# brantburnett/Snappier

Hardware: AMD Instinct MI355X
Metric: uncompressed GB/s block compress+decompress, 64 KiB blocks (higher is better)
Workload: dtype u8

## Files before the change

### snappier_amd/csrc/decode_chains.hip

```cpp
#include "decode_common.h"

#define SNP_MARK(name) asm volatile("; MARK " #name)

#ifndef SNP_DC_FINISH_MIN
#define SNP_DC_FINISH_MIN 1
#endif

namespace {

constexpr u32 kR = 32;
constexpr u32 kW = SNP_WAVE * kR;
constexpr u32 kCap = 128;
constexpr u32 kModeBatch = 0, kModeWindow = 1, kModeLongLiteral = 2, kModeLeave = 3;
constexpr u32 kHist = 64;
constexpr u32 kStage = 2048;

__device__ __forceinline__ u32 adv4(u32 x)
{
    const u32 k1 = 0x01010101u;
    const u32 t = x & 0x03030303u;
    const u32 t1 = t >> 1;
    const u32 hp = ((x >> 2) & 0x3f3f3f3fu) + 0x02020202u;
    const u32 ca = t + k1 + (t1 & t & k1);
    const u32 nz = ((t | t1) & k1) * 255u;
    return (ca & nz) | (hp & ~nz);
}

__device__ __forceinline__ u32x4 adv16(u32x4 v) { return u32x4{adv4(v.x), adv4(v.y), adv4(v.z), adv4(v.w)}; }

__device__ __forceinline__ u32 long_literal_advance(const u8* at, u32 a)
{
    const u32 ex = a - 61u;
    const u32 b1234 = ld32u(at + 1);
    const u32 tr = ex >= 4 ? b1234 : __builtin_amdgcn_ubfe(b1234, 0u, 8 * ex);
    return 2u + ex + min(tr, 0x3fffffffu);
}

__device__ __forceinline__ void store_first_piece(u8* d, u32x4 p0, u32 len)
{
    if (len >= 16u) {
        st128u(d, p0);
    } else {
        const bool c8 = (len & 8u) != 0, c4 = (len & 4u) != 0, c2 = (len & 2u) != 0;
        const u32 a0 = c8 ? p0.z : p0.x;
        const u32 a1 = c8 ? p0.w : p0.y;
        const u32 b0 = c4 ? a1 : a0;
        const u32 c0 = c2 ? b0 >> 16 : b0;
        if (c8) st64u(d, p0.x, p0.y);
        if (c4) st32u(d + (len & 8u), a0);
        if (c2) st16u(d + (len & 12u), b0);
        if (len & 1u) d[len & 14u] = static_cast<u8>(c0);
    }
}

__device__ __forceinline__ void load_pieces(const u8* s, u32 len, bool any_mid, u32x4& p0, u32x4& p1, u32x4& p2, u32x4& p3)
{
    p0 = ld128u(s);
    if (len > 16u) p1 = ld128u(s + len - 16);
    if (any_mid) {
        if (len > 32u) {
            p2 = ld128u(s + 16);
            p3 = ld128u(s + min(32u, len - 16u));
        }
    }
}

__device__ __forceinline__ void store_pieces(u8* d, u32 len, bool any_mid, const u32x4& p0, const u32x4& p1, const u32x4& p2, const u32x4& p3)
{
    store_first_piece(d, p0, len);
    if (len > 16u) st128u(d + len - 16, p1);
    if (any_mid) {
        if (len > 32u) {
            st128u(d + 16, p2);
            if (len > 48u) st128u(d + 32, p3);
        }
    }
}

template <bool FENCED, bool FRAG>
__device__ __forceinline__ void chains_front(DecBlk& B, const u32 lane)
{
    __shared__ __attribute__((aligned(16))) u8 c_tab[kW + 64];
    __shared__ __attribute__((aligned(16))) u8 c_stage_h[kHist + kStage + 64];
    __shared__ u64 c_busy[65];
    u8* const c_stage = c_stage_h + kHist;
    u32* const c_T = reinterpret_cast<u32*>(c_busy);
    u16* const c_pos = reinterpret_cast<u16*>(c_tab);
    const u8* const src = B.src;
    u8* const dst = B.dst;
    const u32 n = B.n, expected = B.expected;
    const u32 skip = FRAG ? B.skip : 0u;
    u32 op = B.op;
    const u32 r0 = kR * lane;
    u32 wbase = B.ip, ntok = 0, emitted = 0, consumed = 0;
    u32 q_pf = 0;
    u32 pf_at = ~0u;
    bool h_valid = false;
    u64 h_pend = 0;
    u32 h_pk = 0, h_op = 0, h_span = 0, h_hist = 0;
    auto finish_held = [&](const bool fence) __attribute__((always_inline)) {
        lanes_sync_lds();
        if (h_pend) {
            if (FENCED && fence) asm volatile("s_waitcnt vmcnt(0)" ::: "memory");
            const u32 vbase = lane + static_cast<u32>(reinterpret_cast<uintptr_t>(c_stage));
            const u32 vbase0 = vbase - lane;
            (void)vbase0;
            u64 pend = h_pend;
            while (pend) {
                u32 f, k;
#if SNP_DC_FINISH_MIN
                {
                    u32 t0, t1, t2, va, vb, vi;
                    asm volatile(
                        "1:\n\t"
                        "s_ff1_i32_b64 %[f], %[pend]\n\t"
                        "v_readlane_b32 %[k], %[pk], %[f]\n\t"
                        "s_bitset0_b64 %[pend], %[f]\n\t"
                        "s_cmp_lt_i32 %[k], 0\n\t"
                        "s_cbranch_scc1 2f\n\t"
                        "s_bfe_u32 %[t0], %[k], 0x7000b\n\t"
                        "s_lshr_b32 %[t1], %[k], 18\n\t"
                        "s_and_b32 %[t2], %[k], 0x7ff\n\t"
                        "v_min_u32_e32 %[vi], %[t0], %[lane]\n\t"
                        "v_add3_u32 %[va], %[vi], %[t1], %[vsrc]\n\t"
                        "ds_read_u8 %[vb], %[va]\n\t"
                        "v_add3_u32 %[va], %[vi], %[t2], %[vbase]\n\t"
                        "s_waitcnt lgkmcnt(0)\n\t"
                        "ds_write_b8 %[va], %[vb]\n\t"
                        "s_cmp_lg_u64 %[pend], 0\n\t"
                        "s_cbranch_scc1 1b\n\t"
                        "2:"
                        : [pend] "+s"(pend), [f] "=&s"(f), [k] "=&s"(k), [t0] "=&s"(t0), [t1] "=&s"(t1), [t2] "=&s"(t2),
                          [va] "=&v"(va), [vb] "=&v"(vb), [vi] "=&v"(vi)
                        : [pk] "v"(h_pk), [lane] "v"(lane), [vbase] "v"(vbase0), [vsrc] "v"(vbase0 - kHist)
                        : "scc", "memory");
#else
                {
                    u32 t0, t1, t2, va, vb;
                    u64 sv;
                    asm volatile(
                        "1:\n\t"
                        "s_ff1_i32_b64 %[f], %[pend]\n\t"
                        "v_readlane_b32 %[k], %[pk], %[f]\n\t"
                        "s_bitset0_b64 %[pend], %[f]\n\t"
                        "s_cmp_lt_i32 %[k], 0\n\t"
                        "s_cbranch_scc1 2f\n\t"
                        "s_bfe_u32 %[t0], %[k], 0x7000b\n\t"
                        "s_lshr_b32 %[t1], %[k], 18\n\t"
                        "s_and_b32 %[t2], %[k], 0x7ff\n\t"
                        "v_cmp_gt_u32_e32 vcc, %[t0], %[lane]\n\t"
                        "s_and_saveexec_b64 %[sv], vcc\n\t"
                        "v_add_u32_e32 %[va], %[t1], %[vsrc]\n\t"
                        "ds_read_u8 %[vb], %[va]\n\t"
                        "v_add_u32_e32 %[va], %[t2], %[vbase]\n\t"
                        "s_waitcnt lgkmcnt(0)\n\t"
                        "ds_write_b8 %[va], %[vb]\n\t"
                        "s_mov_b64 exec, %[sv]\n\t"
                        "s_cmp_lg_u64 %[pend], 0\n\t"
                        "s_cbranch_scc1 1b\n\t"
                        "2:"
                        : [pend] "+s"(pend), [f] "=&s"(f), [k] "=&s"(k), [t0] "=&s"(t0), [t1] "=&s"(t1), [t2] "=&s"(t2), [sv] "=&s"(sv),
                          [va] "=&v"(va), [vb] "=&v"(vb)
                        : [pk] "v"(h_pk), [lane] "v"(lane), [vbase] "v"(vbase), [vsrc] "v"(vbase - kHist)
                        : "vcc", "scc", "memory");
#endif
                    if (static_cast<i32>(k) >= 0) break;
                }
                const u32 f_d = k & 0x7ffu, f_len = ((k >> 11) & 0x7fu) + (SNP_DC_FINISH_MIN ? 1u : 0u);
                const u32 f_off = (k >> 18) & 0x1fffu;
                const u32 sidx = f_off < f_len ? lane_mod(lane, f_off) : lane;
                const u32 spos = f_d + sidx - f_off;
                u32 byte = 0;
                if (__builtin_expect(static_cast<i32>(f_d - f_off) >= -static_cast<i32>(h_hist), 1)) {
                    if (lane < f_len) byte = c_stage[static_cast<i32>(spos)];
                } else {
                    const bool below = static_cast<i32>(spos) < -static_cast<i32>(h_hist);
                    if ((lane < f_len) & !below) byte = c_stage[static_cast<i32>(spos)];
                    if ((lane < f_len) & below) byte = dst[h_op + spos];
                    asm volatile("" : "+v"(byte));
                }
                if (lane < f_len) c_stage[f_d + lane] = static_cast<u8>(byte);
                lanes_sync_lds();
            }
        }
    };
    auto write_out_held = [&]() __attribute__((always_inline)) {
        lanes_sync_lds();
        u8* const g = dst + h_op;
        if (FRAG && h_op < skip) {
            for (u32 i = skip - h_op + lane; i < h_span; i += SNP_WAVE) g[i] = c_stage[i];
        } else {
            for (u32 i = lane * 16; i < h_span; i += SNP_WAVE * 16)
                *reinterpret_cast<snp_u128_unaligned*>(g + i) = *reinterpret_cast<const snp_u128_unaligned*>(c_stage + i);
        }
    };
    for (;;) {
        u32 mode = emitted == ntok ? kModeWindow : kModeBatch;
        u32 len = 0, off = 0, drel = 0, ne = 0, incl = 0, body = 0, s_first = 0, s_len0 = 0, s_body0 = 0, taken = 0;
        bool is_lit = false, live = true;
        if (mode == kModeBatch) {
SNP_MARK(B_top);
            const u32 t = emitted + lane;
            bool have = t < ntok;
            const u32 pos = c_pos[have ? t : emitted];
            u32 q = q_pf;
            if (pf_at != emitted) {
                q = ld32u(src + wbase + pos);
                asm volatile("" : "+v"(q));
            }
            const u32 c = q & 0xffu;
            const u32 type = c & 3u;
            const u32 hi6 = c >> 2;
            u32 b1234 = q >> 8;
            if (__builtin_expect(ballot64(have & ((type == 3u) | (c == 0xfcu))) != 0ull, 0)) {
                if ((type == 3u) | (c == 0xfcu)) b1234 |= static_cast<u32>(src[wbase + pos + 4u]) << 24;
            }
            is_lit = type == 0;
            const bool long_lit = is_lit && hi6 >= 60;
            const u32 extra = is_lit ? (long_lit ? hi6 - 59 : 0u) : (type == 3 ? 4u : type);
            const u32 trailer = extra >= 4 ? b1234 : __builtin_amdgcn_ubfe(b1234, 0u, 8 * extra);
            len = (long_lit ? trailer : (hi6 & (type == 1 ? 7u : 63u))) + (type == 1 ? 4u : 1u);
            off = is_lit ? 0u : (type == 1 ? (((c >> 5) << 8) | (b1234 & 0xffu)) : trailer);
            body = pos + 1u + extra;
            u64 last = ~0ull;
            u32 len_tag0 = 0;
            bool dealt = false;
            if (!FRAG && __builtin_expect(ballot64((q & 0xc0ffu) == 0x40f0u) != 0ull, 0)) {
                const bool two = have && is_lit && len > 64u && len <= 128u;
                dealt = true;
                len_tag0 = read_lane(len, 0);
                const u32 cnt = have ? (two ? 2u : 1u) : 0u;
                const u32 sincl = wave_inclusive_scan(cnt);
                const u32 s0 = sincl - cnt;
                const bool fits = have && sincl <= SNP_WAVE;
                const u32 nslots = read_lane(sincl, static_cast<u32>(__builtin_popcountll(ballot64(fits))) - 1u);
                if (fits) c_busy[s0] = (two ? 64u : min(len, 255u)) | (two ? 0u : 0x100u) | (is_lit ? 0x200u : 0u) | (static_cast<u64>(body) << 10) | (static_cast<u64>(off) << 26);
                if (fits && two) c_busy[s0 + 1u] = (len - 64u) | 0x100u | 0x200u | (static_cast<u64>(body + 64u) << 10);
                lanes_sync_lds();
                const u64 w = c_busy[lane];
                lanes_sync_lds();
                have = lane < nslots;
                len = static_cast<u32>(w) & 0xffu;
                is_lit = (w & 0x200u) != 0;
                body = static_cast<u32>(w >> 10) & 0xffffu;
                off = static_cast<u32>(w >> 26);
                last = ballot64(have && (w & 0x100u) != 0) | ~ballot64(have);
            }
            const u32 olen = have ? len : 0u;
            incl = wave_inclusive_scan(olen);
            drel = incl - olen;
            const u32 room = n - wbase - 16u;
            const bool lit_ok = ((len - 1u) < room) & (body <= room - len);
            const bool dead = FRAG && op + incl <= skip;
            live = !FRAG || op + drel >= skip;
            const bool copy_ok = (off - 1u) < op + drel - skip;
            const bool ok = have & (dead ? (!is_lit | lit_ok) : live & ((is_lit & lit_ok) | (!is_lit & copy_ok))) & (incl + 16u <= expected - op);
            const bool big = is_lit & (len > 64u);
            const u64 okm = ballot64(ok & !big & (incl <= kStage));
            ne = okm == ~0ull ? 64u : static_cast<u32>(__builtin_ctzll(~okm));
            taken = ne;
            if (dealt) {
                if (ne && !((last >> (ne - 1u)) & 1ull)) ne -= 1u;
                taken = static_cast<u32>(__builtin_popcountll(last & (ne == 64u ? ~0ull : (1ull << ne) - 1ull)));
            }
SNP_MARK(B_ne0);
            if (ne == 0) {
                const u32 body0 = read_lane(body, 0);
                const bool long0 = dealt && read_lane(is_lit ? 1u : 0u, 0) != 0u && len_tag0 > 64u;
                const bool whole_ok = (len_tag0 - 1u) < room && body0 <= room - len_tag0 && static_cast<u64>(len_tag0) + 16u <= expected - op;
                const u32 f0 = long0 ? (whole_ok ? 3u : 0u) : read_lane((ok ? 1u : 0u) | (big ? 2u : 0u), 0);
                mode = f0 == 3u ? kModeLongLiteral : kModeLeave;
                s_first = read_lane(pos, 0);
                s_len0 = dealt ? len_tag0 : read_lane(len, 0);
                s_body0 = read_lane(body, 0) | (FRAG && read_lane(dead ? 1u : 0u, 0) ? 0x80000000u : 0u);
            }
        }
        if (mode != kModeBatch) {
            if (h_valid) {
                finish_held(true);
                write_out_held();
                h_valid = false;
            }
            if (mode == kModeLeave) {
                wbase += s_first;
                consumed = 0;
                break;
            }
            if (mode == kModeLongLiteral) {
                if (!FRAG || static_cast<i32>(s_body0) >= 0) wave_copy(dst + op, src + wbase + (s_body0 & 0x7fffffffu), s_len0, lane);
                op += s_len0;
                emitted += 1;
                continue;
            }
SNP_MARK(S_stage_table);
            wbase += consumed;
            consumed = 0;
            if (wbase + 72 > n || op >= expected) break;
            const u32 avail = n - wbase;
            const u32 L = min(kW, avail) - 8u;
            const u8* const wsrc = src + wbase;
            {
                const u32 oa = lane * 16u, ob = oa + 1024u;
                const u32 la = min(oa, avail - 16u), lb = min(ob, avail - 16u);
                const u32x4 va = ld128u(wsrc + la), vb = ld128u(wsrc + lb);
                st128u(c_tab + la, adv16(va));
                st128u(c_tab + lb, adv16(vb));
                lanes_sync_lds();
                c_tab[L + lane] = 64;
            }
            lanes_sync_lds();
SNP_MARK(A_walk);
            u32 p = r0, V = 0, a = 0;
            const u32 lim = min(r0 + kR, L);
            while (p < lim) {
                a = c_tab[p];
                c_tab[p] = static_cast<u8>(a | 0x80u);
                V |= 1u << (p & 31u);
                p += a;
            }
SNP_MARK(Aprime_walk);
            c_T[lane] = 0;
            u32* const c_O = reinterpret_cast<u32*>(c_stage + 512) + lane * (kCap / 32);
#pragma unroll
            for (u32 w = 0; w < kCap / 32; ++w) c_O[w] = 0;
            lanes_sync_lds();
            const bool stopA = (p > r0) & (a >= 62u);
            p = stopA ? p - a : min(p, L + 63u);
            const u32 obase = p & ~(kR - 1u);
            u32* const c_Ob = c_O - (obase >> 5);
            a = c_tab[p];
            u32 x = a | ((p - obase) & ~(kCap - 1u));
            while (x < 62u) {
                atomicOr(&c_Ob[p >> 5], 1u << (p & 31u));
                p += a;
                a = c_tab[p];
                x = a | ((p - obase) & ~(kCap - 1u));
            }
            const u32 nx = stopA ? 65u : (a & 0x80u) ? p >> 5 : (p >= L ? 64u : 65u);
SNP_MARK(R_reach);
            const u32 m = p;
            u64 active;
            u32 entry = 0;
            {
                u8* const c_reach = c_stage;
                u32* const c_entry = reinterpret_cast<u32*>(c_stage + SNP_WAVE);
                u32 hop = nx;
                bool reached = lane == 0;
                c_reach[lane] = reached ? 1 : 0;
#pragma unroll
                for (int k = 0; k < 6; ++k) {
                    lanes_sync_lds();
                    if (reached && hop < 64u) c_reach[hop] = 1;
                    lanes_sync_lds();
                    reached = c_reach[lane] != 0;
                    const u32 h2 = bperm(hop, hop);
                    hop = hop < 64u ? h2 : hop;
                }
                if (reached && nx < 64u) c_entry[nx] = m;
                lanes_sync_lds();
                if (lane) entry = c_entry[lane];
                lanes_sync_lds();
                active = ballot64(reached);
                const u64 ends = ballot64(reached && nx == 64u);
                consumed = ends ? read_lane(m, static_cast<u32>(__builtin_ctzll(ends))) : 0u;
            }
            if (ballot64(((active >> lane) & 1ull) && nx == 65u)) {
                active = 0;
                entry = 0;
                for (u32 k = 0, e = 0;;) {
                    active |= 1ull << k;
                    entry = lane == k ? e : entry;
                    u32 mk = read_lane(m, k), nk = read_lane(nx, k);
                    if (nk == 65u) {
                        nk = 64u;
                        for (bool first = true; mk < L; first = false) {
                            u32 a = bcast_first(static_cast<u32>(c_tab[mk]));
                            if (!first && a >= 128u) { nk = mk >> 5; break; }
                            a &= 0x7fu;
                            if (lane == 0) atomicOr(&c_T[mk >> 5], 1u << (mk & 31u));
                            if (a >= 62u) a = bcast_first(long_literal_advance(wsrc + mk, a));
                            mk += a;
                        }
                    }
                    if (nk >= 64u) { consumed = mk; break; }
                    e = mk;
                    k = nk;
                }
            }
SNP_MARK(T_list);
            if ((active >> lane) & 1ull) {
                const u32 own = V & ~((1u << (entry & 31u)) - 1u);
                const u32 w0 = obase >> 5;
                if (own) atomicOr(&c_T[lane], own);
#pragma unroll
                for (u32 w = 0; w < kCap / 32; ++w) {
                    const u32 ow = c_O[w];
                    if (ow && w0 + w < SNP_WAVE) atomicOr(&c_T[w0 + w], ow);
                }
            }
            lanes_sync_lds();
            const u32 Tw = c_T[lane];
            const u32 cnt = static_cast<u32>(__builtin_popcount(Tw));
            const u32 cincl = wave_inclusive_scan(cnt);
            ntok = read_lane(cincl, 63);
            lanes_sync_lds();
            u32 t = cincl - cnt, bits = Tw;
            while (bits) {
                c_pos[t++] = static_cast<u16>(r0 + static_cast<u32>(__builtin_ctz(bits)));
                bits &= bits - 1u;
            }
            lanes_sync_lds();
            emitted = 0;
            pf_at = ~0u;
            if (ntok == 0) {
                consumed = 0;
                break;
            }
            continue;
    }
SNP_MARK(B_pass1);
        const bool act = lane < ne;
        const u32 span = read_lane(incl, ne - 1);
        const u32 gap = h_valid ? op - h_op : 0u;
        const u32 reach = drel + len;
        const u32 back = gap + (h_valid ? h_hist : 0u);
        const bool far = !is_lit & (off >= reach + gap);
        const bool near = act & live & !is_lit & !far & (off >= reach) & (off <= drel + back);
        const bool early = act & live & (is_lit | far);
        const bool waits = act & live & !early & !near;
        if (FENCED) asm volatile("s_waitcnt vmcnt(0)" ::: "memory");
        pf_at = emitted + taken;
        if (pf_at < ntok) q_pf = ld32u(src + wbase + c_pos[pf_at + lane < ntok ? pf_at + lane : pf_at]);
        const bool any_mid = ballot64(act & (len > 32u)) != 0ull;
        const u32 sofs_mine = is_lit ? wbase + body : op + drel - off;
        u32x4 p0, p1, p2, p3;
        if (early) load_pieces((is_lit ? src : dst) + sofs_mine, len, any_mid, p0, p1, p2, p3);
SNP_MARK(B_finish);
        if (h_valid) finish_held(false);
SNP_MARK(B_writeout);
        asm volatile("; loads of the new batch are back"
                     :: "v"(p0.x), "v"(p0.y), "v"(p0.z), "v"(p0.w), "v"(p1.x), "v"(p1.y), "v"(p1.z), "v"(p1.w), "v"(p2.x), "v"(p2.y), "v"(p2.z),
                        "v"(p2.w), "v"(p3.x), "v"(p3.y), "v"(p3.z), "v"(p3.w), "v"(q_pf)
                     : "memory");
        if (h_valid) write_out_held();
SNP_MARK(B_stage);
        if (near) load_pieces(c_stage + static_cast<i32>(drel + gap - off), len, any_mid, p0, p1, p2, p3);
        const u32 hist = h_valid ? min(kHist, h_hist + gap) : 0u;
        if (hist) {
            const u8 hb = c_stage[static_cast<i32>(gap + lane - kHist)];
            if (lane >= kHist - hist) c_stage[static_cast<i32>(lane - kHist)] = hb;
        }
        lanes_sync_lds();
        if (early | near) store_pieces(c_stage + drel, len, any_mid, p0, p1, p2, p3);
        {
            const bool plain = (off >= len) & (off <= drel + hist);
            h_pend = ballot64(waits);
            h_pk = drel | ((len - (SNP_DC_FINISH_MIN ? 1u : 0u)) << 11) | (plain ? (drel - off + kHist) << 18 : 0x80000000u | (off << 18));
            h_op = op;
            h_span = span;
            h_hist = hist;
            h_valid = true;
        }
        op += span;
        emitted += taken;
    }
SNP_MARK(Z_exit);
    B.ip = wbase;
    B.op = op;
    B.w.wv = 0x80000000u;
}

template <bool FENCED, bool FRAG>
__device__ __forceinline__ void decode_block_chains(SNP_D_PARAMS, const u32 b)
{
    const u32 lane = lane_id();
    DecBlk B;
    if (!block_begin<FRAG>(SNP_D_ARGS, b, lane, B)) return;
    if (B.st == SNP_OK) chains_front<FENCED, FRAG>(B, lane);
    serial_tail<FENCED, FRAG>(B, b, lane, out_len, status);
}

#ifdef SNP_DC_VGPRS
#define SNP_DC_ATTR __attribute__((amdgpu_waves_per_eu(8, 8), amdgpu_num_vgpr(SNP_DC_VGPRS)))
#else
#define SNP_DC_ATTR __attribute__((amdgpu_waves_per_eu(8, 8)))
#endif
template <bool FENCED>
__global__ __launch_bounds__(SNP_WAVE) SNP_DC_ATTR void k_decode_chains(SNP_D_PARAMS)
{
    decode_block_chains<FENCED, false>(SNP_D_ARGS, blockIdx.x);
}

template <bool FENCED>
__global__ __launch_bounds__(SNP_WAVE) SNP_DC_ATTR void k_decode_chains_frag(SNP_D_PARAMS)
{
    decode_block_chains<FENCED, true>(SNP_D_ARGS, blockIdx.x);
}

template <bool FENCED>
__global__ __launch_bounds__(SNP_WAVE) SNP_DC_ATTR void k_decode_chains_list(
    SNP_D_PARAMS, const u32* __restrict__ list, u32* __restrict__ ctl, u32 sub_cap)
{
    const u32 lane = lane_id();
    const u32 mine = __hip_atomic_load(&ctl[lane], __ATOMIC_RELAXED, __HIP_MEMORY_SCOPE_AGENT);
    const u32 incl = wave_inclusive_scan(mine);
    const u32 count = read_lane(incl, 63);
    const u32 grab = min(max(count / (gridDim.x * 8u), 1u), 64u);
    for (u32 first = blockIdx.x * grab; first < count;) {
        const u32 last = min(first + grab, count);
        for (u32 i = first; i < last; ++i) {
            const u32 sub = static_cast<u32>(__builtin_popcountll(ballot64(incl <= i)));
            const u32 before = read_lane(incl - mine, sub);
            decode_block_chains<FENCED, false>(SNP_D_ARGS, list[static_cast<u64>(sub) * sub_cap + (i - before)]);
            asm volatile("s_waitcnt vmcnt(0) lgkmcnt(0)" ::: "memory");
        }
        u32 next = 0;
        if (lane == 0) next = atomicAdd(&ctl[64], grab);
        first = gridDim.x * grab + bcast_first(next);
    }
}

}

extern "C" hipError_t snp_launch_decode_chains(const u8* in, const u64* in_off, const u32* in_len, u32 nblocks, u8* out, const u64* out_off,
                                               const u32* out_cap, u32* out_len, i32* status, const u8* chunk_type, int fenced, int redo_only,
                                               unsigned lds_bytes, hipStream_t stream, const u32* frag_skip)
{
    if (nblocks == 0) return hipSuccess;
    if (frag_skip) {
        if (fenced)
            hipLaunchKernelGGL((k_decode_chains_frag<true>), dim3(nblocks), dim3(SNP_WAVE), lds_bytes, stream, in, in_off, in_len, nblocks, out, out_off,
                               out_cap, out_len, status, nullptr, frag_skip, 0);
        else
            hipLaunchKernelGGL((k_decode_chains_frag<false>), dim3(nblocks), dim3(SNP_WAVE), lds_bytes, stream, in, in_off, in_len, nblocks, out, out_off,
                               out_cap, out_len, status, nullptr, frag_skip, 0);
        return hipGetLastError();
    }
    const u32* const no_skip = nullptr;
    if (fenced)
        hipLaunchKernelGGL((k_decode_chains<true>), dim3(nblocks), dim3(SNP_WAVE), lds_bytes, stream, in, in_off, in_len, nblocks, out, out_off,
                           out_cap, out_len, status, chunk_type, no_skip, redo_only);
    else
        hipLaunchKernelGGL((k_decode_chains<false>), dim3(nblocks), dim3(SNP_WAVE), lds_bytes, stream, in, in_off, in_len, nblocks, out, out_off,
                           out_cap, out_len, status, chunk_type, no_skip, redo_only);
    return hipGetLastError();
}

extern "C" hipError_t snp_launch_decode_chains_list(const u8* in, const u64* in_off, const u32* in_len, u32 nblocks, u8* out, const u64* out_off,
                                                    const u32* out_cap, u32* out_len, i32* status, const u8* chunk_type, int fenced,
                                                    unsigned lds_bytes, hipStream_t stream, const u32* list, u32* ctl, u32 waves, u32 sub_cap)
{
    if (nblocks == 0) return hipSuccess;
    const u32* const no_skip = nullptr;
    if (fenced)
        hipLaunchKernelGGL((k_decode_chains_list<true>), dim3(waves), dim3(SNP_WAVE), lds_bytes, stream, in, in_off, in_len, nblocks, out, out_off,
                           out_cap, out_len, status, chunk_type, no_skip, 0, list, ctl, sub_cap);
    else
        hipLaunchKernelGGL((k_decode_chains_list<false>), dim3(waves), dim3(SNP_WAVE), lds_bytes, stream, in, in_off, in_len, nblocks, out, out_off,
                           out_cap, out_len, status, chunk_type, no_skip, 0, list, ctl, sub_cap);
    return hipGetLastError();
}
```

Measured before the change: 92.31.

## Compact pending copy descriptors by rank and walk them with an unrolled loop

Pending copy descriptors are repacked into a new bit layout and compacted with ds_permute, so entry i of the pending set sits in lane i. The finish loop can then walk lanes 0..w-1 in order with an inline-asm loop unrolled by two. This replaces the per-entry find-first-set and bit-clear scalar work. Slow (overlapping) entries are found with a ballot and handled by a shared fallback routine. It adds a permute per batch, narrows the offset field from 13 to 12 bits, and relies on the compaction keeping the original ordering.

Measured after the change: 76.58. 17.0% lower.

```diff
diff --git a/snappier_amd/csrc/decode_chains.hip b/snappier_amd/csrc/decode_chains.hip
--- a/snappier_amd/csrc/decode_chains.hip
+++ b/snappier_amd/csrc/decode_chains.hip
@@ -3,7 +3,7 @@
 #define SNP_MARK(name) asm volatile("; MARK " #name)
 
 #ifndef SNP_DC_FINISH_MIN
-#define SNP_DC_FINISH_MIN 1
+#define SNP_DC_FINISH_MIN 2
 #endif
 
 namespace {
@@ -98,17 +98,82 @@
     bool h_valid = false;
     u64 h_pend = 0;
     u32 h_pk = 0, h_op = 0, h_span = 0, h_hist = 0;
+    auto finish_slow = [&](const u32 f_d, const u32 f_len, const u32 f_off) __attribute__((always_inline)) {
+        const u32 sidx = f_off < f_len ? lane_mod(lane, f_off) : lane;
+        const u32 spos = f_d + sidx - f_off;
+        u32 byte = 0;
+        if (__builtin_expect(static_cast<i32>(f_d - f_off) >= -static_cast<i32>(h_hist), 1)) {
+            if (lane < f_len) byte = c_stage[static_cast<i32>(spos)];
+        } else {
+            const bool below = static_cast<i32>(spos) < -static_cast<i32>(h_hist);
+            if ((lane < f_len) & !below) byte = c_stage[static_cast<i32>(spos)];
+            if ((lane < f_len) & below) byte = dst[h_op + spos];
+            asm volatile("" : "+v"(byte));
+        }
+        if (lane < f_len) c_stage[f_d + lane] = static_cast<u8>(byte);
+        lanes_sync_lds();
+    };
     auto finish_held = [&](const bool fence) __attribute__((always_inline)) {
         lanes_sync_lds();
         if (h_pend) {
             if (FENCED && fence) asm volatile("s_waitcnt vmcnt(0)" ::: "memory");
             const u32 vbase = lane + static_cast<u32>(reinterpret_cast<uintptr_t>(c_stage));
             const u32 vbase0 = vbase - lane;
+            (void)vbase;
             (void)vbase0;
+#if SNP_DC_FINISH_MIN == 2
+            const u32 w = static_cast<u32>(__builtin_popcountll(h_pend));
+            __builtin_assume(w != 0u);
+            u64 slow = ballot64(static_cast<i32>(h_pk) < 0);
+            auto plain_run = [&](u32& i, const u32 e) __attribute__((always_inline)) {
+                u32 k, t1, t2, va, vb, vi;
+                asm volatile(
+                    "s_sub_u32 %[t1], %[e], %[i]\n\t"
+                    "s_bitcmp1_b32 %[t1], 0\n\t"
+                    "s_cbranch_scc1 2f\n\t"
+                    "1:\n\t"
+                    "v_readlane_b32 %[k], %[pk], %[i]\n\t"
+                    "s_add_u32 %[i], %[i], 1\n\t"
+                    "s_bfe_u32 %[t1], %[k], 0xc0008\n\t"
+                    "s_lshr_b32 %[t2], %[k], 20\n\t"
+                    "v_min_u32_sdwa %[vi], %[k], %[lane] dst_sel:DWORD dst_unused:UNUSED_PAD src0_sel:BYTE_0 src1_sel:DWORD\n\t"
+                    "v_add3_u32 %[va], %[vi], %[t1], %[vsrc]\n\t"
+                    "ds_read_u8 %[vb], %[va]\n\t"
+                    "v_add3_u32 %[va], %[vi], %[t2], %[vbase]\n\t"
+                    "s_waitcnt lgkmcnt(0)\n\t"
+                    "ds_write_b8 %[va], %[vb]\n\t"
+                    "2:\n\t"
+                    "v_readlane_b32 %[k], %[pk], %[i]\n\t"
+                    "s_add_u32 %[i], %[i], 1\n\t"
+                    "s_bfe_u32 %[t1], %[k], 0xc0008\n\t"
+                    "s_lshr_b32 %[t2], %[k], 20\n\t"
+                    "v_min_u32_sdwa %[vi], %[k], %[lane] dst_sel:DWORD dst_unused:UNUSED_PAD src0_sel:BYTE_0 src1_sel:DWORD\n\t"
+                    "v_add3_u32 %[va], %[vi], %[t1], %[vsrc]\n\t"
+                    "ds_read_u8 %[vb], %[va]\n\t"
+                    "v_add3_u32 %[va], %[vi], %[t2], %[vbase]\n\t"
+                    "s_waitcnt lgkmcnt(0)\n\t"
+                    "ds_write_b8 %[va], %[vb]\n\t"
+                    "s_cmp_lt_u32 %[i], %[e]\n\t"
+                    "s_cbranch_scc1 1b"
+                    : [i] "+s"(i), [k] "=&s"(k), [t1] "=&s"(t1), [t2] "=&s"(t2), [va] "=&v"(va), [vb] "=&v"(vb), [vi] "=&v"(vi)
+                    : [e] "s"(e), [pk] "v"(h_pk), [lane] "v"(lane), [vbase] "v"(vbase0), [vsrc] "v"(vbase0 - kHist)
+                    : "scc", "memory");
+            };
+            u32 i = 0;
+            while (__builtin_expect(slow != 0ull, 0)) {
+                const u32 e = static_cast<u32>(__builtin_ctzll(slow));
+                if (i < e) plain_run(i, e);
+                const u32 k = read_lane(h_pk, e);
+                finish_slow((k >> 20) & 0x7ffu, (k & 0x7fu) + 1u, (k >> 8) & 0xfffu);
+                slow &= ~(1ull << e);
+                i = e + 1u;
+            }
+            if (i < w) plain_run(i, w);
+#else
             u64 pend = h_pend;
             while (pend) {
                 u32 f, k;
-#if SNP_DC_FINISH_MIN
+#if SNP_DC_FINISH_MIN == 1
                 {
                     u32 t0, t1, t2, va, vb, vi;
                     asm volatile(
@@ -166,22 +231,10 @@
 #endif
                     if (static_cast<i32>(k) >= 0) break;
                 }
-                const u32 f_d = k & 0x7ffu, f_len = ((k >> 11) & 0x7fu) + (SNP_DC_FINISH_MIN ? 1u : 0u);
-                const u32 f_off = (k >> 18) & 0x1fffu;
-                const u32 sidx = f_off < f_len ? lane_mod(lane, f_off) : lane;
-                const u32 spos = f_d + sidx - f_off;
-                u32 byte = 0;
-                if (__builtin_expect(static_cast<i32>(f_d - f_off) >= -static_cast<i32>(h_hist), 1)) {
-                    if (lane < f_len) byte = c_stage[static_cast<i32>(spos)];
-                } else {
-                    const bool below = static_cast<i32>(spos) < -static_cast<i32>(h_hist);
-                    if ((lane < f_len) & !below) byte = c_stage[static_cast<i32>(spos)];
-                    if ((lane < f_len) & below) byte = dst[h_op + spos];
-                    asm volatile("" : "+v"(byte));
-                }
-                if (lane < f_len) c_stage[f_d + lane] = static_cast<u8>(byte);
-                lanes_sync_lds();
-            }
+                const u32 f_len = ((k >> 11) & 0x7fu) + (SNP_DC_FINISH_MIN ? 1u : 0u);
+                finish_slow(k & 0x7ffu, f_len, (k >> 18) & 0x1fffu);
+            }
+#endif
         }
     };
     auto write_out_held = [&]() __attribute__((always_inline)) {
@@ -455,7 +508,17 @@
         {
             const bool plain = (off >= len) & (off <= drel + hist);
             h_pend = ballot64(waits);
+#if SNP_DC_FINISH_MIN == 2
+            h_pk = (len - 1u) | (drel << 20) | (plain ? (drel - off + kHist) << 8 : 0x80000000u | (off << 8));
+#else
             h_pk = drel | ((len - (SNP_DC_FINISH_MIN ? 1u : 0u)) << 11) | (plain ? (drel - off + kHist) << 18 : 0x80000000u | (off << 18));
+#endif
+#if SNP_DC_FINISH_MIN == 2
+            if (h_pend) {
+                const u32 rank = __builtin_amdgcn_mbcnt_hi(static_cast<u32>(h_pend >> 32), __builtin_amdgcn_mbcnt_lo(static_cast<u32>(h_pend), 0u));
+                h_pk = static_cast<u32>(__builtin_amdgcn_ds_permute(static_cast<int>((waits ? rank : 63u) << 2), static_cast<int>(waits ? h_pk : 0u)));
+            }
+#endif
             h_op = op;
             h_span = span;
             h_hist = hist;
```
